# amazon-science/siam-mot

Hardware: AMD Instinct MI355X
Metric: frame-pairs/sec at 720p, 30 active tracks; EMM xcorr HBM GB/s vs peak (higher is better)
Workload: dtype f32 (towers and correlation: fp16x2 operands on MFMA, fp32 accumulate, fp32-equivalent error); 1 GPU; EMM tracker-head frame pair (EMM.forward + EMM.extract_cache) on DLA-34-FPN 720p FPN maps (net input 704x1280, C=128, 5 levels), 30 tracks, one stream per GPU; hot path only: backbone / RPN / box head / solver are outside the timed region; tracks=30, channels=128, rz=15, rx=30, feature_sets=8, feature_bytes_rotated=307281920

## Files before the change

measure/debug/tower_stage_timeline.py:

```python
import json, os, sys
import numpy as np, torch
sys.path.insert(0, os.path.join(os.path.dirname(__file__), "..", "..")); sys.path.insert(0, os.path.join(os.path.dirname(__file__), "..", "..", "tests"))
import golden_inputs as gi
import siammot_amd.ops as ops
dev = "cuda:0"
rs = np.random.RandomState(0)
Pn = gi.predictor_params(rs, 128, np.array([[0, 0, 80, 120]], dtype=np.float32))
P = {k: torch.from_numpy(v).to(dev) for k, v in Pn.items()}
n = int(os.environ.get("TRACKS", "30"))
resp = torch.randn(n, 128, 16, 16, device=dev) * 15
with ops.debug_library(SMOT_TOWER_OCT=2, SMOT_TOWER_BF3=1, SMOT_WINO_ABL=15):
    f = lambda: ops.emm_predictor(resp, P)
    for _ in range(20): f()
    torch.cuda.synchronize()
    grid = (n + 7) // 8 * 8 * 8
    tr = torch.zeros(grid * 64, dtype=torch.int64, device=dev)
    lib = ops.load_library()
    lib.smot_debug_trace(ops._ptr(tr)); f(); torch.cuda.synchronize(); tr.zero_(); f(); torch.cuda.synchronize()
    lib.smot_debug_trace(ops._ptr(None))
t = tr.view(grid, 8, 8).cpu().numpy().astype(np.float64)
t = t[t[:, 0, 5] != 0]
base = t[:, :, 0].min(axis=1)[:, None, None]
rel = (t[:, :, :6] - base)
names = ["before_barrier1", "after_barrier1", "raw_planes_stored", "vector_phase_done", "after_vmcnt0_and_barrier2", "matrix_and_fetches_issued"]
print(json.dumps({"tracks": n, "workgroups": int(t.shape[0]), "slots": names,
                  "mean_cycles_by_wave": {("wave%d" % w): [round(float(x), 0) for x in rel[:, w, :].mean(0)] for w in range(8)}}))
```

measure/debug/tower_wg_spread.py:

```python
import json, os, sys
import numpy as np, torch
sys.path.insert(0, os.path.join(os.path.dirname(__file__), "..", "..")); sys.path.insert(0, os.path.join(os.path.dirname(__file__), "..", "..", "tests"))
import golden_inputs as gi
import siammot_amd.ops as ops
dev = "cuda:0"
rs = np.random.RandomState(0)
P = {k: torch.from_numpy(v).to(dev) for k, v in gi.predictor_params(rs, 128, np.array([[0, 0, 80, 120]], dtype=np.float32)).items()}
for n in [int(t) for t in os.environ.get("TRACKS", "30").split(",")]:
    resp = torch.randn(n, 128, 16, 16, device=dev) * 15
    with ops.debug_library(SMOT_TOWER_OCT=2, SMOT_TOWER_BF3=1):
        f = lambda: ops.emm_predictor(resp, P)
        for _ in range(30): f()
        torch.cuda.synchronize()
        grid = (n + 7) // 8 * 8 * 8
        tr = torch.zeros(grid * 8, dtype=torch.int64, device=dev)
        lib = ops.load_library()
        lib.smot_debug_trace(ops._ptr(tr))
        rows = []
        for rep in range(5):
            tr.zero_(); f(); torch.cuda.synchronize()
            t = tr.view(grid, 8).cpu().numpy().astype(np.float64); t = t[t[:, 5] != 0]
            t0 = t[:, 0].min()
            rows.append({"workgroups": int(t.shape[0]), "start_offset_mean": float((t[:, 0] - t0).mean()), "start_offset_max": float((t[:, 0] - t0).max()),
                         "duration_mean": float((t[:, 5] - t[:, 0]).mean()), "duration_min": float((t[:, 5] - t[:, 0]).min()), "duration_max": float((t[:, 5] - t[:, 0]).max()),
                         "first_start_to_last_end": float(t[:, 5].max() - t0),
                         "phase_max": [float(x) for x in np.diff(t[:, :6], axis=1).max(0)], "phase_p90": [float(x) for x in np.percentile(np.diff(t[:, :6], axis=1), 90, axis=0)]})
        lib.smot_debug_trace(ops._ptr(None))
        ts = []
        for rep in range(3):
            ops.kernel_timer_begin(ops.TIMER_TOWER, 200)
            for _ in range(200): f()
            ms, cnt = ops.kernel_timer_end(ops.TIMER_TOWER)
            ts.append(ms / cnt * 1e3)
    print(json.dumps({"tracks": n, "tower_us": round(min(ts), 2), "launches": rows[-2:]}))
```

measure/lib_ab.py:

```python
import json, os, sys
import torch
sys.path.insert(0, os.path.join(os.path.dirname(os.path.abspath(__file__)), ".."))
import bench
import siammot_amd.ops as ops
from siammot_amd.structures import BoxList
from siammot_amd.emm import EMM
from siammot_amd.config import get_default_cfg
from siammot_amd.track_utils import build_track_utils
dev = torch.device("cuda:0")
base = ops.load_library()
other = ops._open(os.path.abspath(sys.argv[1]), ops._SIGNATURES)
assert other.smot_abi_version() == ops.ABI_VERSION
feats = [bench.synthetic_features(k, dev) for k in range(4)]
n = 30
boxes = bench.synthetic_boxes(n, (1280, 704)).to(dev)
det = BoxList(boxes, (1280, 704), mode="xyxy")
det.add_field("ids", torch.arange(n, device=dev))
det.add_field("labels", torch.ones(n, dtype=torch.int64, device=dev))
cfg = get_default_cfg(channels=bench.CHANNELS)
emm = EMM(cfg, build_track_utils(cfg)).eval()
bench.init_predictor(emm.predictor, boxes.cpu())
emm = emm.to(dev)
ref = None
for rep in range(3):
    for name, lib in (("product", base), ("variant", other)):
        ops._lib = lib
        with torch.no_grad():
            state = emm.extract_cache(feats[3], det)
            def step(k, state):
                z, sr, d = state
                _, res, _ = emm(feats[k % 4], d, sr, template_features=z)
                return emm.extract_cache(feats[k % 4], det), res
            for k in range(100):
                state, res = step(k, state)
            out = torch.cat((res[0].bbox, res[0].get_field("scores")[:, None]), 1).clone()
            ref = out if ref is None else ref
            torch.cuda.synchronize()
            ts = []
            for _ in range(5):
                e0, e1 = torch.cuda.Event(enable_timing=True), torch.cuda.Event(enable_timing=True)
                e0.record()
                for k in range(300):
                    state, res = step(k, state)
                e1.record(); torch.cuda.synchronize()
                ts.append(e0.elapsed_time(e1) / 300 * 1e3)
            r = bench.tracking_loop_throughput(30, dev, feats[:2], steps=400, refine=True)
        print(json.dumps({"library": name, "frame_pair_us": round(min(ts), 2), "bitwise_equal": bool(torch.equal(out, ref)),
                          "loop_refine_ms": round(r["ms_per_frame"], 4)}), flush=True)
ops._lib = base
```

siam-mot_amd/csrc/tower_wino.hip:

```cpp
#include "tower_common.h"
#include "knobs.h"
#include <utility>

namespace smot {

constexpr int W_ROW = 24;
constexpr int W_PLANE = 448;
constexpr int W_STAGE_IC = 8;
constexpr int W_RING = 4;
constexpr int W_BUF = W_STAGE_IC * W_PLANE;
constexpr int W_XOC = 68;
constexpr int W_X_FLOATS = 4 * 2 * 16 * W_XOC;
constexpr int W_PL_OFF = W_X_FLOATS;
constexpr int W_HW_OFF = W_PL_OFF + 16 * T_PLANE;
constexpr int W_ST_OFF = W_HW_OFF + 16 * 36;
constexpr int W_EPI_FLOATS = W_ST_OFF + 32;
constexpr int w_smem_floats(int oct) {
    return (oct * W_EPI_FLOATS > W_RING * W_BUF) ? oct * W_EPI_FLOATS : W_RING * W_BUF;
}
constexpr int W_A_FLOATS = 4 * 4 * 2 * 2 * 256;
constexpr int W_A_SLOT = 4 * 2 * 2 * 256;
constexpr int W_AB_ROW = 4 * 2 * 1024;
static_assert((W_RING * W_BUF + W_A_FLOATS) * 4 <= 160 * 1024, "BF3: ring + A image in one CU's LDS");
static_assert(w_smem_floats(1) * 4 <= 64 * 1024, "OCT = 1: two workgroups per CU, no opt-in needed");
static_assert(w_smem_floats(2) * 4 <= 160 * 1024, "OCT = 2: one workgroup per CU");

__device__ __forceinline__ float tower_pack_scale(unsigned wmax_bits) {
    const int e = (int)((wmax_bits >> 23) & 0xffu);
    if (e == 0 || e == 255) return 1.0f;
    int k = 266 - e;
    k = k < 1 ? 1 : (k > 254 ? 254 : k);
    return __uint_as_float((unsigned)k << 23);
}

__global__ void __launch_bounds__(256)
tower_pack_kernel(const float* __restrict__ wc, const float* __restrict__ wr, int C, float* __restrict__ packed,
                  unsigned* __restrict__ hdr) {
    const int idx = blockIdx.x * 256 + threadIdx.x;
    if (idx >= 2 * C * C) return;
    const int oc = idx / C, ic = idx - oc * C;
    const float* g = (oc < C ? wc + (size_t)oc * C * 9 : wr + (size_t)(oc - C) * C * 9) + (size_t)ic * 9;
    float gg[4][3];
#pragma unroll
    for (int v = 0; v < 3; ++v) {
        const float g0 = g[v], g1 = g[3 + v], g2 = g[6 + v];
        gg[0][v] = g0;
        gg[1][v] = 0.5f * ((g0 + g1) + g2);
        gg[2][v] = 0.5f * ((g0 - g1) + g2);
        gg[3][v] = g2;
    }
    const int tile = oc >> 4, k = ic >> 2, lane = (oc & 15) + 16 * (ic & 3);
    const int nk = C >> 2;
#pragma unroll
    for (int i = 0; i < 4; ++i) {
        float4 u;
        u.x = gg[i][0];
        u.y = 0.5f * ((gg[i][0] + gg[i][1]) + gg[i][2]);
        u.z = 0.5f * ((gg[i][0] - gg[i][1]) + gg[i][2]);
        u.w = gg[i][2];
        *reinterpret_cast<float4*>(packed + ((((size_t)tile * nk + k) * 4 + i) * 64 + lane) * 4) = u;
        if ((C & 31) == 0) {
            unsigned short* hf = reinterpret_cast<unsigned short*>(packed + (size_t)2 * C * C * 16);
            const int kb = ic >> 5, sidx = (ic & 31) >> 2, nkb1 = (C >> 5) + 1;
            const float su = tower_pack_scale(hdr[0]);
            const float uq[4] = {u.x, u.y, u.z, u.w};
#pragma unroll
            for (int q = 0; q < 4; ++q) {
                const int kbp = ((sidx >> 1) <= q) ? kb : kb + 1;
                float r = uq[q] * su;
#pragma unroll
                for (int part = 0; part < 2; ++part) {
                    const _Float16 h = (_Float16)r;
                    r -= (float)h;
                    hf[((((((size_t)tile * nkb1 + kbp) * 4 + i) * 4 + q) * 2 + part) * 64 + lane) * 8 + sidx] =
                        __builtin_bit_cast(unsigned short, h);
                }
            }
            if (idx == 0 && i == 0) reinterpret_cast<float*>(hdr)[1] = 1.0f / su;
        }
    }
}

__global__ void __launch_bounds__(256)
tower_wmax_kernel(const float* __restrict__ wc, const float* __restrict__ wr, int count, unsigned* __restrict__ hdr) {
    float m = 0.0f;
    for (int e = blockIdx.x * 256 + threadIdx.x; e < count; e += gridDim.x * 256) m = fmaxf(m, fmaxf(fabsf(wc[e]), fabsf(wr[e])));
    for (int off = 32; off; off >>= 1) m = fmaxf(m, __shfl_xor(m, off));
    if ((threadIdx.x & 63) == 0) atomicMax(hdr, __float_as_uint(m));
}

__global__ void __launch_bounds__(256)
plane_absmax_kernel(const float* __restrict__ resp, int planes, int hw, float* __restrict__ pm) {
    const int plane = blockIdx.x * 4 + (threadIdx.x >> 6), lane = threadIdx.x & 63;
    if (plane >= planes) return;
    const float* __restrict__ src = resp + (size_t)plane * hw;
    float m = 0.0f;
    for (int e = lane; e < hw; e += 64) m = plane_max_step(m, src[e]);
    m = plane_max_wave(m);
    if (lane == 0) pm[plane] = m;
}

int launch_plane_absmax(const float* resp, int planes, int hw, float* pm, hipStream_t st) {
    hipLaunchKernelGGL(plane_absmax_kernel, dim3((planes + 3) / 4), dim3(256), 0, st, resp, planes, hw, pm);
    return check_launch("predictor towers (plane maxima)");
}

template <int G, int... E>
__device__ __forceinline__ void heads_group(const float (&hw)[9], const float (&a)[36], f32x4& h0, f32x4& h1,
                                            std::integer_sequence<int, E...>) {
    (((E % 2 == 0 ? h0 : h1) = __builtin_amdgcn_mfma_f32_4x4x1f32(hw[(G * 36 + E) / 16], a[E], (E % 2 == 0 ? h0 : h1), 4,
                                                                  (G * 36 + E) % 16, 0)), ...);
}

template <int ABL, int OCT, int BHO = 0, bool BF3 = false>
__global__ void __launch_bounds__(256 * OCT, OCT == 1 ? 2 : 1)
tower_wino_kernel(const float* __restrict__ resp, const float* __restrict__ packed, const float* __restrict__ plane_max,
                  unsigned* __restrict__ zero_words, long long* __restrict__ trace, int N, int C, int cpg, float eps,
                  float* __restrict__ part, TowerParams P) {
    constexpr int NT = 256 * OCT;
    constexpr int NP = 2 / OCT;
    constexpr bool BLOCKED = BHO > 0;
    constexpr int MAP = BLOCKED ? BHO * BHO : 256;
    constexpr int RAW4 = 512 / NT;
    constexpr int RAWB = (W_STAGE_IC * 324 + NT - 1) / NT;
    static_assert(!BLOCKED || (BHO > 16 && BHO <= 32), "four 16 x 16 blocks cover maps of 17 .. 32");
    extern __shared__ __attribute__((aligned(16))) float sm[];
    const int tid = threadIdx.x;
#define W_TRACE(SLOT) \
    if (ABL != 15 && trace && tid == 0) trace[(size_t)blockIdx.x * 8 + (SLOT)] = (long long)__builtin_amdgcn_s_memtime();
    W_TRACE(0)
    if (ABL != 15 && trace && tid == 0) {
        trace[(size_t)blockIdx.x * 8 + 6] = (long long)__builtin_amdgcn_s_getreg(0xF804);
        trace[(size_t)blockIdx.x * 8 + 7] = (long long)__builtin_amdgcn_s_getreg(0xF814);
    }
    const int lane = tid & 63;
    const int wave = __builtin_amdgcn_readfirstlane(tid >> 6);
    const int xi = wave & 3;
    const int nh = wave >> 2;
    const int tiles_per_tower = C >> 4;
    const int tiles = 2 * tiles_per_tower;
    const int wg_per_track = tiles / OCT;
    const int xcd = blockIdx.x & 7, slot = blockIdx.x >> 3;
    const int wg_per_n = BLOCKED ? 4 * wg_per_track : wg_per_track;
    const int n = (slot / wg_per_n) * 8 + xcd;
    const int within = slot % wg_per_n;
    const int blk = BLOCKED ? within / wg_per_track : 0;
    const int oy = BLOCKED ? (blk >> 1) * (BHO - 16) : 0, ox = BLOCKED ? (blk & 1) * (BHO - 16) : 0;
    const int tile0 = (within % wg_per_track) * OCT;
    if (n >= N) return;
    if (zero_words != nullptr && tile0 == 0 && blk == 0 && tid == 0) zero_words[n] = 0u;
    const float* __restrict__ in = resp + (size_t)n * C * MAP;
    const int nk = C >> 2;
    const int nstages = C / W_STAGE_IC;
    const int sub = tid >> 8, ltid = tid & 255;
    const int etile = tile0 + sub;
    const int tower = etile / tiles_per_tower;
    const int oc0 = (etile - tower * tiles_per_tower) * 16;

    auto make_rsrc = [](const float* base) {
        const unsigned long long a = reinterpret_cast<unsigned long long>(base);
        const unsigned lo = __builtin_amdgcn_readfirstlane((unsigned)a);
        const unsigned hi = __builtin_amdgcn_readfirstlane((unsigned)(a >> 32));
        return __builtin_amdgcn_make_buffer_rsrc(reinterpret_cast<void*>(((unsigned long long)hi << 32) | lo), 0,
                                                 0x7fffffff, 0x00020000);
    };
    typedef unsigned u32x4 __attribute__((ext_vector_type(4)));
    auto make_rsrc_sized = [](const float* base, unsigned bytes) {
        const unsigned long long a = reinterpret_cast<unsigned long long>(base);
        const unsigned lo = __builtin_amdgcn_readfirstlane((unsigned)a);
        const unsigned hi = __builtin_amdgcn_readfirstlane((unsigned)(a >> 32));
        return __builtin_amdgcn_make_buffer_rsrc(reinterpret_cast<void*>(((unsigned long long)hi << 32) | lo), 0,
                                                 (int)bytes, 0x00020000);
    };
    const auto rs_in = BLOCKED ? make_rsrc_sized(in, (unsigned)C * MAP * 4u) : make_rsrc(in);
    const auto rs_a = make_rsrc(packed);
    constexpr int NRAW = BLOCKED ? (RAWB + 3) / 4 : RAW4;
    float4 prs[2][NRAW];
    unsigned raw_voff[BLOCKED ? RAWB : RAW4];
    int raw_lds[BLOCKED ? RAWB : RAW4];
    if constexpr (!BLOCKED) {
#pragma unroll
        for (int j = 0; j < RAW4; ++j) {
            const int f = tid + NT * j;
            const int f4 = f & 63;
            raw_voff[j] = (unsigned)((f >> 6) * 256 + f4 * 4) * 4u;
            raw_lds[j] = (f >> 6) * W_PLANE + ((f4 >> 2) + 1) * W_ROW + 1 + (f4 & 3) * 4;
        }
    } else {
#pragma unroll
        for (int j = 0; j < RAWB; ++j) {
            const int e = tid + NT * j;
            const int ch = e / 324, rem = e - ch * 324;
            const int r = rem / 18, c = rem - r * 18;
            const int sy = oy - 1 + r, sx = ox - 1 + c;
            const bool inside = e < W_STAGE_IC * 324 && sy >= 0 && sy < BHO && sx >= 0 && sx < BHO;
            raw_voff[j] = inside ? (unsigned)(ch * MAP + sy * BHO + sx) * 4u : 0x7FFF0000u;
            raw_lds[j] = e < W_STAGE_IC * 324 ? ch * W_PLANE + r * W_ROW + c : (W_STAGE_IC - 1) * W_PLANE + 432 + (tid & 15);
        }
    }
    auto load_raw = [&](int st, float4* pr) {
        const int soff = __builtin_amdgcn_readfirstlane(st * (W_STAGE_IC * MAP * 4));
        if constexpr (!BLOCKED) {
#pragma unroll
            for (int j = 0; j < RAW4; ++j) {
                const u32x4 v = __builtin_bit_cast(u32x4, __builtin_amdgcn_raw_buffer_load_b128(rs_in, raw_voff[j], soff, 0));
                pr[j] = make_float4(__uint_as_float(v.x), __uint_as_float(v.y), __uint_as_float(v.z), __uint_as_float(v.w));
            }
        } else {
            float* f = reinterpret_cast<float*>(pr);
#pragma unroll
            for (int j = 0; j < RAWB; ++j)
                f[j] = __int_as_float(__builtin_amdgcn_raw_buffer_load_b32(rs_in, raw_voff[j], soff, 0));
        }
    };
    typedef int i32x4 __attribute__((ext_vector_type(4)));
    const unsigned long long pin = reinterpret_cast<unsigned long long>(in);
    const i32x4 rs_in_words = {__builtin_amdgcn_readfirstlane((int)(unsigned)pin),
                               __builtin_amdgcn_readfirstlane((int)((unsigned)(pin >> 32) & 0xffffu)),
                               BLOCKED ? (int)((unsigned)C * MAP * 4u) : 0x7fffffff, 0x00020000};
    auto load_raw_asm = [&](int st, float4* pr) __attribute__((always_inline)) {
        const int soff = __builtin_amdgcn_readfirstlane(st * (W_STAGE_IC * MAP * 4));
        if constexpr (!BLOCKED) {
#pragma unroll
            for (int j = 0; j < RAW4; ++j) {
                f32x4 v;
                asm volatile("buffer_load_dwordx4 %0, %1, %2, %3 offen" : "=v"(v) : "v"(raw_voff[j]), "s"(rs_in_words), "s"(soff) : "memory");
                pr[j] = make_float4(v[0], v[1], v[2], v[3]);
            }
        } else {
            float* f = reinterpret_cast<float*>(pr);
#pragma unroll
            for (int j = 0; j < RAWB; ++j)
                asm volatile("buffer_load_dword %0, %1, %2, %3 offen" : "=v"(f[j]) : "v"(raw_voff[j]), "s"(rs_in_words), "s"(soff) : "memory");
        }
    };
    float sv = 1.0f, inv_sv = 1.0f;
    auto store_raw = [&](float* buf, const float4* pr) {
        if constexpr (!BLOCKED) {
#pragma unroll
            for (int j = 0; j < RAW4; ++j) {
                float* d = buf + raw_lds[j];
                d[0] = BF3 ? pr[j].x * sv : pr[j].x;
                d[1] = BF3 ? pr[j].y * sv : pr[j].y;
                d[2] = BF3 ? pr[j].z * sv : pr[j].z;
                d[3] = BF3 ? pr[j].w * sv : pr[j].w;
            }
        } else {
            const float* f = reinterpret_cast<const float*>(pr);
#pragma unroll
            for (int j = 0; j < RAWB; ++j) buf[raw_lds[j]] = BF3 ? f[j] * sv : f[j];
        }
    };
    const unsigned a_voff = (unsigned)lane * 16u;
    const int a_base = __builtin_amdgcn_readfirstlane((int)((((size_t)tile0 * nk) * 4 + xi) * 1024));
    const int a_tile = nk * 4096;
    f32x4 aset[2][2][OCT];
    auto load_a = [&](int st, f32x4 (*dst)[OCT]) {
#pragma unroll
        for (int o = 0; o < OCT; ++o)
#pragma unroll
            for (int k = 0; k < 2; ++k) {
                const int soff = __builtin_amdgcn_readfirstlane(a_base + o * a_tile + (2 * st + k) * 4096);
                dst[k][o] = __builtin_bit_cast(f32x4, __builtin_amdgcn_raw_buffer_load_b128(rs_a, a_voff, soff, 0));
            }
    };

    const int nkb = C >> 5;
    const int ab_block = 4 * W_AB_ROW;
    const int ab_base = __builtin_amdgcn_readfirstlane(2 * C * C * 64 + ((tile0 + nh) * (nkb + 1) * 4 + xi) * W_AB_ROW);
    typedef __attribute__((address_space(3))) float lds_float;
    lds_float* const a_lds = (lds_float*)(sm + W_RING * W_BUF);
    const int al_wave = __builtin_amdgcn_readfirstlane((xi * 2 + nh) * 512);
    const int al_row = __builtin_amdgcn_readfirstlane(xi * 2 * 512);
    const unsigned long long pa = reinterpret_cast<unsigned long long>(packed);
    const i32x4 rs_a_words = {__builtin_amdgcn_readfirstlane((int)(unsigned)pa),
                              __builtin_amdgcn_readfirstlane((int)((unsigned)(pa >> 32) & 0xffffu)), 0x7fffffff, 0x00020000};
    const unsigned a_lds_byte = (unsigned)(size_t)a_lds;
    auto dma_part = [&](int q, int kbp, int part) __attribute__((always_inline)) {
        const int soff = __builtin_amdgcn_readfirstlane(ab_base + (ABL == 12 ? 0 : kbp) * ab_block + (q * 2 + part) * 1024);
        const unsigned dst = __builtin_amdgcn_readfirstlane(a_lds_byte + (unsigned)(q * W_A_SLOT + al_wave + part * 256) * 4u);
        unsigned keep;
        asm volatile("s_mov_b32 %0, m0\n\ts_mov_b32 m0, %1\n\ts_nop 0\n\tbuffer_load_dwordx4 %2, %3, %4 offen lds\n\ts_mov_b32 m0, %0"
                     : "=&s"(keep) : "s"(dst), "v"(a_voff), "s"(rs_a_words), "s"(soff) : "memory");
    };
    auto dma_slot = [&](int q, int kbp) __attribute__((always_inline)) {
        dma_part(q, kbp, 0);
        dma_part(q, kbp, 1);
    };
    auto load_al = [&](int q, u32x4 (*dst)[2]) __attribute__((always_inline)) {
        const float* src = sm + W_RING * W_BUF + q * W_A_SLOT + al_row + lane * 4;
#pragma unroll
        for (int o = 0; o < OCT; ++o)
#pragma unroll
            for (int part = 0; part < 2; ++part)
                dst[o][part] = *reinterpret_cast<const u32x4*>(src + (o * 2 + part) * 256);
    };
    f32x4 acc[OCT][4][2 * NP];
#pragma unroll
    for (int o = 0; o < OCT; ++o)
#pragma unroll
        for (int q = 0; q < 4; ++q)
#pragma unroll
            for (int t = 0; t < 2 * NP; ++t) acc[o][q][t] = (f32x4){0.f, 0.f, 0.f, 0.f};

    load_raw(0, prs[0]);
    load_raw(1, prs[1]);
    if constexpr (BF3) {
        dma_slot(0, 0);
        dma_slot(1, 0);
    }
    if constexpr (!BF3) load_a(0, aset[0]);
    if (ABL == 2 || ABL >= 5) {
#pragma unroll
        for (int o = 0; o < OCT; ++o) {
            aset[1][0][o] = aset[0][0][o];
            aset[1][1][o] = aset[0][1][o];
        }
    }
    float pmv[2] = {0.0f, 0.0f};
    if constexpr (BF3 && ABL != 10) {
        const float* __restrict__ pmsrc = plane_max + (size_t)n * C;
        if (lane < C) pmv[0] = pmsrc[lane];
        if (lane + 64 < C) pmv[1] = pmsrc[lane + 64];
        __builtin_amdgcn_sched_barrier(0);
    }
    {
        float4* z = reinterpret_cast<float4*>(sm);
        for (int e = tid; e < W_RING * W_BUF / 4; e += NT) z[e] = make_float4(0.f, 0.f, 0.f, 0.f);
    }
    float hwv[9];
    auto load_hwv = [&]() __attribute__((always_inline)) {
        const int o = lane & 3, blk = lane >> 2;
        const float* wsrc = (tower == 1) ? P.reg_w + (size_t)o * C * 9
                                         : (o < 2 ? P.cls_w + (size_t)o * C * 9 : P.center_w);
        const bool live = (tower == 1) || (o < 3);
        wsrc += (size_t)oc0 * 9 + blk;
#pragma unroll
        for (int r = 0; r < 9; ++r) hwv[r] = live ? wsrc[r * 16] : 0.0f;
    };
    if constexpr (!BF3) load_hwv();
    if constexpr (BF3 && ABL != 10) {
        float m = fmaxf(pmv[0], pmv[1]);
        for (int c = lane + 128; c < C; c += 64) m = fmaxf(m, plane_max[(size_t)n * C + c]);
        m = plane_max_wave(m);
        const int e = (int)((__float_as_uint(m) >> 23) & 0xffu);
        if (e != 0 && e != 255) {
            int k = 139 - e;
            k = k < -100 ? -100 : (k > 100 ? 100 : k);
            sv = __uint_as_float((unsigned)(127 + k) << 23);
            inv_sv = __uint_as_float((unsigned)(127 - k) << 23);
        }
    }

    __syncthreads();
    if constexpr (BF3) asm volatile("s_waitcnt vmcnt(0)" ::: "memory");
    store_raw(sm, prs[0]);
    store_raw(sm + W_BUF, prs[1]);
    load_raw(min(2, nstages - 1), prs[0]);
    load_raw(min(3, nstages - 1), prs[1]);
    float ga = 0.0f, be = 0.0f;
    if constexpr (!BLOCKED) {
        ga = P.gamma[tower][oc0 + (ltid >> 4)];
        be = P.beta[tower][oc0 + (ltid >> 4)];
    }
    __syncthreads();

    const int row_a = (xi == 0) ? 0 : ((xi == 2) ? 2 : 1);
    const int row_b = (xi == 2) ? 1 : ((xi == 3) ? 3 : 2);
    const int kq = lane >> 4, xl = lane & 15;
    const int patch0 = kq * W_PLANE + (2 * (xl >> 2) + (OCT == 2 ? 8 * nh : 0)) * W_ROW + 4 * (xl & 3);
    int ia = patch0 + row_a * W_ROW, ib = patch0 + row_b * W_ROW;
    asm volatile("" : "+v"(ia), "+v"(ib));

    float rd[NP][6][2];
    float bop[4][2 * NP];
    if (ABL >= 3) {
#pragma unroll
        for (int e = 0; e < 12 * NP; ++e) {
            (&bop[0][0])[e % (8 * NP)] = (float)(lane + e);
            (&rd[0][0][0])[e] = (float)(lane - e);
        }
    }
#define W_READ(BUFI, Q, RD)                                                                      \
    if (ABL != 3 && (ABL < 5 || ABL >= 7)) {                                                     \
        const float* oa = sm + ia + ((BUFI) * W_BUF + (Q) * 4 * W_PLANE);                        \
        const float* ob = sm + ib + ((BUFI) * W_BUF + (Q) * 4 * W_PLANE);                        \
        _Pragma("unroll") for (int p = 0; p < NP; ++p) {             \
            f32x4 a4 = *reinterpret_cast<const f32x4*>(oa + p * 8 * W_ROW);                      \
            f32x2 a2 = *reinterpret_cast<const f32x2*>(oa + p * 8 * W_ROW + 4);                  \
            f32x4 b4 = *reinterpret_cast<const f32x4*>(ob + p * 8 * W_ROW);                      \
            f32x2 b2 = *reinterpret_cast<const f32x2*>(ob + p * 8 * W_ROW + 4);                  \
            if (BF3) asm volatile("" : "+v"(a4), "+v"(a2), "+v"(b4), "+v"(b2));                  \
            RD[p][0][0] = a4[0]; RD[p][0][1] = b4[0];                                            \
            RD[p][1][0] = a4[1]; RD[p][1][1] = b4[1];                                            \
            RD[p][2][0] = a4[2]; RD[p][2][1] = b4[2];                                            \
            RD[p][3][0] = a4[3]; RD[p][3][1] = b4[3];                                            \
            RD[p][4][0] = a2[0]; RD[p][4][1] = b2[0];                                            \
            RD[p][5][0] = a2[1]; RD[p][5][1] = b2[1];                                            \
        }                                                                                        \
    }
#define W_XFORM(RD, BOP)                                                                         \
    if (ABL != 3 && (ABL < 5 || ABL >= 7)) _Pragma("unroll") for (int p = 0; p < NP; ++p) {      \
                     \
        float w[6];                                                                              \
        _Pragma("unroll") for (int c = 0; c < 6; ++c)                                            \
            w[c] = PLUS ? RD[p][c][0] + RD[p][c][1] : RD[p][c][0] - RD[p][c][1];                 \
        BOP[0][2 * p] = w[0] - w[2];                                                             \
        BOP[1][2 * p] = w[1] + w[2];                                                             \
        BOP[2][2 * p] = w[2] - w[1];                                                             \
        BOP[3][2 * p] = w[1] - w[3];                                                             \
        BOP[0][2 * p + 1] = w[2] - w[4];                                                         \
        BOP[1][2 * p + 1] = w[3] + w[4];                                                         \
        BOP[2][2 * p + 1] = w[4] - w[3];                                                         \
        BOP[3][2 * p + 1] = w[3] - w[5];                                                         \
    }
#define W_MFMA(AV, BOP)                                                                          \
    if (ABL != 4) _Pragma("unroll") for (int t = 0; t < 2 * NP; ++t)                             \
        _Pragma("unroll") for (int o = 0; o < OCT; ++o) {                                        \
            acc[o][0][t] = __builtin_amdgcn_mfma_f32_16x16x4f32(AV[o][0], BOP[0][t], acc[o][0][t], 0, 0, 0);   \
            acc[o][1][t] = __builtin_amdgcn_mfma_f32_16x16x4f32(AV[o][1], BOP[1][t], acc[o][1][t], 0, 0, 0);   \
            acc[o][2][t] = __builtin_amdgcn_mfma_f32_16x16x4f32(AV[o][2], BOP[2][t], acc[o][2][t], 0, 0, 0);   \
            acc[o][3][t] = __builtin_amdgcn_mfma_f32_16x16x4f32(AV[o][3], BOP[3][t], acc[o][3][t], 0, 0, 0);   \
        }
#define W_FENCE __builtin_amdgcn_sched_barrier(0);
#define W_STAGE(J)                                                                               \
    {                                                                                            \
        if (ABL != 6) __syncthreads();                                                           \
        if (ABL != 1 && ABL < 5) store_raw(sm + (((J) + 2) & 3) * W_BUF, prs[(J) & 1]);          \
        if (ABL != 1 && ABL < 5) load_raw(min(s0 + (J) + 4, nstages - 1), prs[(J) & 1]);         \
        if (ABL != 2 && ABL < 5) load_a(min(s0 + (J) + 1, nstages - 1), aset[((J) + 1) & 1]);    \
        W_FENCE                                                                                  \
        W_READ((J), 1, rd)                                                      \
        W_MFMA(aset[(J) & 1][0], bop)                                                            \
        W_FENCE                                                                                  \
        W_XFORM(rd, bop)                                                                         \
        W_FENCE                                                                                  \
        W_READ(((J) + 1) & 3, 0, rd)                     \
        W_MFMA(aset[(J) & 1][1], bop)                                                            \
        W_FENCE                                                                                  \
        W_XFORM(rd, bop)                                                                         \
        W_FENCE                                                                                  \
    }
#define W_LOOP                                                                                   \
    W_READ(0, 0, rd)                                                                             \
    W_XFORM(rd, bop)                                                                             \
    W_FENCE                                                                                      \
    for (int s0 = 0; s0 < nstages; s0 += 4) {        \
        W_STAGE(0)                                                                               \
        W_STAGE(1)                                                                               \
        W_STAGE(2)                                                                               \
        W_STAGE(3)                                                                               \
    }
    typedef _Float16 f16x2 __attribute__((ext_vector_type(2)));
    typedef _Float16 f16x4 __attribute__((ext_vector_type(4)));
    typedef _Float16 f16x8 __attribute__((ext_vector_type(8)));
    typedef unsigned u32x2 __attribute__((ext_vector_type(2)));
    u32x4 Bp[2][4][2];
    float rdb[NP][6][2];
    if constexpr (BF3) {
#pragma unroll
        for (int e = 0; e < 16; ++e) (&Bp[0][0][0])[e] = (u32x4){0u, 0u, 0u, 0u};
    }
    const f16x4 negI = __builtin_bit_cast(f16x4, (u32x2){(lane & 3) == 0 ? 0x0000BC00u : ((lane & 3) == 1 ? 0xBC000000u : 0u),
                                                         (lane & 3) == 2 ? 0x0000BC00u : ((lane & 3) == 3 ? 0xBC000000u : 0u)});
#define WB_CVT(D, A, B) D = __builtin_bit_cast(unsigned, __builtin_convertvector((f32x2){A, B}, f16x2));
#define WB_SPLIT(J, BA, BB)                                                                      \
    {                                                                                            \
        f32x4 v4[4];                                                                             \
        unsigned hh[4][2], mm[4][2];                                                             \
        _Pragma("unroll") for (int q = 0; q < 4; ++q) {                                          \
            v4[q] = (f32x4){BA[q][0], BB[q][0], BA[q][1], BB[q][1]};                             \
            WB_CVT(hh[q][0], v4[q][0], v4[q][1]) WB_CVT(hh[q][1], v4[q][2], v4[q][3])            \
        }                                                                                        \
        W_FENCE                                                                                  \
        _Pragma("unroll") for (int q = 0; q < 4; ++q)                                            \
            v4[q] = __builtin_amdgcn_mfma_f32_4x4x4f16(negI, __builtin_bit_cast(f16x4, (u32x2){hh[q][0], hh[q][1]}), v4[q], 0, 0, 0); \
        W_FENCE                                                                                  \
        _Pragma("unroll") for (int q = 0; q < 4; ++q) {                                          \
            WB_CVT(mm[q][0], v4[q][0], v4[q][1]) WB_CVT(mm[q][1], v4[q][2], v4[q][3])            \
        }                                                                                        \
        W_FENCE                                                                                  \
        _Pragma("unroll") for (int q = 0; q < 4; ++q) {                                          \
            Bp[0][q][0][J] = hh[q][0]; Bp[0][q][1][J] = hh[q][1];                                \
            Bp[1][q][0][J] = mm[q][0]; Bp[1][q][1][J] = mm[q][1];                                \
        }                                                                                        \
    }
#define WB_MM(O, Q, T, PA, PB)                                                                   \
    if (ABL != 7) acc[O][Q][T] = __builtin_amdgcn_mfma_f32_16x16x32_f16(__builtin_bit_cast(f16x8, AB[O][PA]), \
                                                          __builtin_bit_cast(f16x8, Bp[PB][Q][T]), acc[O][Q][T], 0, 0, 0);
#define WB_TERM(Q, PA, PB) WB_MM(0, Q, 0, PA, PB) WB_MM(1, Q, 0, PA, PB) WB_MM(0, Q, 1, PA, PB) WB_MM(1, Q, 1, PA, PB)
#define WB_Q(Q)                                                                                  \
    {                                                                                            \
        u32x4 AB[OCT][2];                                                                        \
        load_al(Q, AB);                                                                          \
        WB_QM(Q)                                                                                 \
    }
#define WB_QM(Q)                                                                                 \
    {                                                                                            \
        if (ABL == 7) { _Pragma("unroll") for (int t = 0; t < 2; ++t) _Pragma("unroll") for (int e = 0; e < 4; ++e)  \
            acc[0][Q][t][e] += __uint_as_float(Bp[0][Q][t][e] ^ Bp[1][Q][t][e] ^ AB[0][0][e] ^ AB[1][1][e]); } \
        WB_TERM(Q, 1, 0) WB_TERM(Q, 0, 1) WB_TERM(Q, 0, 0)                                       \
    }
    const float sgn = __uint_as_float(__builtin_amdgcn_readfirstlane(xi == 1 ? 0x3f800000u : 0xbf800000u));
#define WB_XFORM(RD, BOP)                                                                        \
    _Pragma("unroll") for (int p = 0; p < NP; ++p) {                                             \
        float w[6];                                                                              \
        _Pragma("unroll") for (int c = 0; c < 6; ++c) w[c] = __builtin_fmaf(sgn, RD[p][c][1], RD[p][c][0]); \
        BOP[0][2 * p] = w[0] - w[2];                                                             \
        BOP[1][2 * p] = w[1] + w[2];                                                             \
        BOP[2][2 * p] = w[2] - w[1];                                                             \
        BOP[3][2 * p] = w[1] - w[3];                                                             \
        BOP[0][2 * p + 1] = w[2] - w[4];                                                         \
        BOP[1][2 * p + 1] = w[3] + w[4];                                                         \
        BOP[2][2 * p + 1] = w[4] - w[3];                                                         \
        BOP[3][2 * p + 1] = w[3] - w[5];                                                         \
    }
#define WB_STAMP(J, KB, SLOT) if (ABL == 15 && (KB) == 2 && (J) == 1 && trace && lane == 0) \
        trace[((size_t)blockIdx.x * 8 + wave) * 8 + (SLOT)] = (long long)__builtin_amdgcn_s_memtime();
#define WB_STAGE(J, KB)                                                                          \
    {                                                                                            \
         \
        WB_STAMP(J, KB, 0)                                                                       \
        asm volatile("s_barrier" ::: "memory");                                                  \
        WB_STAMP(J, KB, 1)                                                                       \
        store_raw(sm + (((J) + 2) & 3) * W_BUF, prs[(J) & 1]);                                   \
        W_FENCE                                                                                  \
        WB_STAMP(J, KB, 2)                                                                       \
        float ba[4][2 * NP], bb[4][2 * NP];                                                      \
        u32x4 AB[OCT][2];                                                                        \
        WB_XFORM(rd, ba)                                                          \
        W_READ(((J) + 1) & 3, 0, rd)                     \
        WB_XFORM(rdb, bb)                                                       \
        W_READ(((J) + 1) & 3, 1, rdb)                                                            \
        WB_SPLIT(J, ba, bb)                                                                      \
        load_al(J, AB);                                                                          \
        W_FENCE                                                                                  \
        WB_STAMP(J, KB, 3)                                                                       \
                                            \
        asm volatile("s_waitcnt vmcnt(0) lgkmcnt(12)\n\ts_barrier" ::: "memory");                \
        W_FENCE                                                                                  \
        WB_STAMP(J, KB, 4)                                                                       \
         \
        WB_TERM(J, 1, 0)                                                                         \
        W_FENCE                                                                                  \
        if (ABL != 9) load_raw_asm(min(4 * (KB) + (J) + 4, nstages - 1), prs[(J) & 1]);          \
        if (ABL != 9) dma_part(((J) + 2) & 3, (KB) + ((J) >= 2 ? 1 : 0), 0);                     \
        W_FENCE                                                                                  \
        WB_TERM(J, 0, 1)                                                                         \
        W_FENCE                                                                                  \
        if (ABL != 9) dma_part(((J) + 2) & 3, (KB) + ((J) >= 2 ? 1 : 0), 1);                     \
        W_FENCE                                                                                  \
        WB_TERM(J, 0, 0)                                                                         \
        W_FENCE                                                                                  \
        WB_STAMP(J, KB, 5)                                                                       \
    }
#define WB_BLOCK(KB) WB_STAGE(0, KB) WB_STAGE(1, KB) WB_STAGE(2, KB) WB_STAGE(3, KB)
#define WB_LOOP                                                                                  \
    W_READ(0, 0, rd)                                                                             \
    W_READ(0, 1, rdb)                                                                            \
    if (nh == 1) asm volatile("s_barrier" ::: "memory");             \
    if (nkb == 4) {                      \
        WB_BLOCK(0) WB_BLOCK(1) WB_BLOCK(2) WB_BLOCK(3)                                          \
    } else if ((nkb & 1) == 0) {                      \
        for (int kb = 0; kb < nkb; kb += 2) { WB_BLOCK(kb) WB_BLOCK(kb + 1) }                    \
    } else {                                                                                     \
        for (int kb = 0; kb < nkb; ++kb) { WB_BLOCK(kb) }                                        \
    }                                                                                            \
                                                                      \
    asm volatile("s_barrier" ::: "memory");                                                      \
    dma_slot(2, nkb);                                                                            \
    asm volatile("s_barrier" ::: "memory");                                                      \
    WB_Q(0)                                                                                      \
    asm volatile("s_waitcnt vmcnt(0)" ::: "memory");                                             \
     \
    _Pragma("unroll") for (int j = 0; j < NRAW; ++j) asm volatile("" :: "v"(prs[0][j].x), "v"(prs[0][j].y), "v"(prs[0][j].z), "v"(prs[0][j].w), \
                                                                    "v"(prs[1][j].x), "v"(prs[1][j].y), "v"(prs[1][j].z), "v"(prs[1][j].w)); \
    asm volatile("s_barrier\n\ts_barrier" ::: "memory");                                         \
    WB_Q(1)                                                                                      \
    asm volatile("s_barrier\n\ts_barrier" ::: "memory");                                         \
    WB_Q(2)                                                                                      \
    if (nh == 0) asm volatile("s_barrier" ::: "memory");
    W_TRACE(1)
    if constexpr (BF3) {
        static_assert(!BF3 || (OCT == 2 && (ABL == 0 || ABL == 7 || ABL == 9 || ABL == 10 || ABL == 12 || ABL == 15)), "BF3: two-tile workgroups only");
        {
            WB_LOOP
        }
        load_hwv();
    } else if (xi == 1) {
        constexpr bool PLUS = true;
        W_LOOP
    } else {
        constexpr bool PLUS = false;
        W_LOOP
    }
    __syncthreads();
#undef WB_LOOP
#undef WB_STAGE
#undef WB_STAMP
#undef WB_BLOCK
#undef WB_XFORM
#undef WB_Q
#undef WB_QM
#undef WB_TERM
#undef WB_MM
#undef WB_SPLIT
#undef WB_CVT
#undef W_LOOP
#undef W_FENCE
#undef W_STAGE
#undef W_MFMA
#undef W_XFORM
#undef W_READ
    W_TRACE(2)

#pragma unroll
    for (int o = 0; o < OCT; ++o)
#pragma unroll
        for (int t = 0; t < 2 * NP; ++t)
#pragma unroll
            for (int r = 0; r < 4; ++r) {
                const float p0 = (acc[o][0][t][r] + acc[o][1][t][r]) + acc[o][2][t][r];
                const float p1 = (acc[o][1][t][r] - acc[o][2][t][r]) - acc[o][3][t][r];
                float* dst = sm + o * W_EPI_FLOATS + ((xi * 2) * 16 + (kq * 4 + r)) * W_XOC +
                             16 * (t + (OCT == 2 ? 2 * nh : 0)) + xl;
                dst[0] = p0;
                dst[16 * W_XOC] = p1;
            }
    float* X = sm + sub * W_EPI_FLOATS;
    float* planes = X + W_PL_OFF;
    float* chs = X + W_ST_OFF;
    for (int e = ltid; e < 16 * 68; e += 256) {
        const int pl = e / 68, c = e - pl * 68;
        const int row = c < 18 ? 0 : (c < 36 ? 17 : 1 + ((c - 36) >> 1));
        const int col = c < 18 ? c : (c < 36 ? c - 18 : (((c - 36) & 1) ? 17 : 0));
        planes[pl * T_PLANE + row * 18 + col] = 0.0f;
    }
    __syncthreads();

    W_TRACE(3)
    const int ocl = ltid >> 4, x16 = ltid & 15;
    float y[4][2][2];
#pragma unroll
    for (int b = 0; b < 2; ++b) {
        const float* src = X + (b * 16 + ocl) * W_XOC + 4 * x16;
        const f32x4 x0 = *reinterpret_cast<const f32x4*>(src + 0 * 32 * W_XOC);
        const f32x4 x1 = *reinterpret_cast<const f32x4*>(src + 1 * 32 * W_XOC);
        const f32x4 x2 = *reinterpret_cast<const f32x4*>(src + 2 * 32 * W_XOC);
        const f32x4 x3 = *reinterpret_cast<const f32x4*>(src + 3 * 32 * W_XOC);
#pragma unroll
        for (int t = 0; t < 4; ++t) {
            y[t][0][b] = (x0[t] + x1[t]) + x2[t];
            y[t][1][b] = (x1[t] - x2[t]) - x3[t];
        }
    }
    if constexpr (BF3) {
        const float inv_su = packed[(size_t)2 * C * C * 16 + (size_t)tiles * (nkb + 1) * 8192 + 1];
#pragma unroll
        for (int t = 0; t < 4; ++t)
#pragma unroll
            for (int a = 0; a < 2; ++a)
#pragma unroll
                for (int b = 0; b < 2; ++b) y[t][a][b] = (y[t][a][b] * inv_sv) * inv_su;
    }

    if constexpr (BLOCKED) {
        constexpr int OV = 32 - BHO;
        float* __restrict__ cdst = part + ((size_t)n * 2 * C + (size_t)tower * C + oc0 + ocl) * MAP;
#pragma unroll
        for (int t = 0; t < 4; ++t) {
            const int ty = (x16 & 3) + 4 * (x16 >> 3), tx = 2 * t + ((x16 >> 2) & 1);
#pragma unroll
            for (int a = 0; a < 2; ++a)
#pragma unroll
                for (int b = 0; b < 2; ++b) {
                    const int lr = 2 * ty + a, lc = 2 * tx + b;
                    if ((oy == 0 || lr >= OV) && (ox == 0 || lc >= OV)) cdst[(oy + lr) * BHO + ox + lc] = y[t][a][b];
                }
        }
        return;
    }
    const float inv_cnt = 1.0f / (float)(cpg * 256);
    float s = 0.0f;
#pragma unroll
    for (int t = 0; t < 4; ++t) s += (y[t][0][0] + y[t][0][1]) + (y[t][1][0] + y[t][1][1]);
    s = group16_sum(s);
    float mean = 0.0f, var = 0.0f;
    const int g0 = (ocl / cpg) * cpg;
    if (cpg == 4) {
#define W_RL(V, L) __int_as_float(__builtin_amdgcn_readlane(__float_as_int(V), (L)))
        mean = (((0.0f + W_RL(s, 0)) + W_RL(s, 16)) + W_RL(s, 32)) + W_RL(s, 48);
    } else {
        if (x16 == 0) chs[ocl] = s;
        __syncthreads();
        for (int ch = g0; ch < g0 + cpg; ++ch) mean += chs[ch];
    }
    mean *= inv_cnt;
    float sq = 0.0f;
#pragma unroll
    for (int t = 0; t < 4; ++t)
#pragma unroll
        for (int a = 0; a < 2; ++a)
#pragma unroll
            for (int b = 0; b < 2; ++b) {
                const float d = y[t][a][b] - mean;
                sq += d * d;
            }
    sq = group16_sum(sq);
    if (cpg == 4) {
        var = (((0.0f + W_RL(sq, 0)) + W_RL(sq, 16)) + W_RL(sq, 32)) + W_RL(sq, 48);
#undef W_RL
    } else {
        if (x16 == 0) chs[16 + ocl] = sq;
        __syncthreads();
        for (int ch = g0; ch < g0 + cpg; ++ch) var += chs[16 + ch];
    }
    const float rstd = 1.0f / sqrtf(var * inv_cnt + eps);
    {
        float* pl = planes + ocl * T_PLANE;
#pragma unroll
        for (int t = 0; t < 4; ++t) {
            const int ty = (x16 & 3) + 4 * (x16 >> 3), tx = 2 * t + ((x16 >> 2) & 1);
#pragma unroll
            for (int a = 0; a < 2; ++a)
#pragma unroll
                for (int b = 0; b < 2; ++b) {
                    float v = (y[t][a][b] - mean) * rstd * ga + be;
                    pl[(2 * ty + a + 1) * 18 + 2 * tx + b + 1] = relu_nan(v);
                }
        }
    }
    __syncthreads();

    W_TRACE(4)
    {
        const int py = ((ltid >> 6) << 1) + ((ltid >> 5) & 1) + (((ltid >> 4) & 1) << 3), px = ltid & 15;
        const float* pl0 = planes + py * 18 + px;
        f32x4 hacc = {0.0f, 0.0f, 0.0f, 0.0f}, hacc1 = {0.0f, 0.0f, 0.0f, 0.0f};
        float av[2][36];
#define W_HLOAD(G, BUF) _Pragma("unroll") for (int e = 0; e < 36; ++e)                                        \
        av[BUF][e] = pl0[((G) * 4 + e / 9) * T_PLANE + ((e % 9) / 3) * 18 + (e % 9) % 3];
#define W_HMM(G, BUF) heads_group<G>(hwv, av[BUF], hacc, hacc1, std::make_integer_sequence<int, 36>{});
        W_HLOAD(0, 0)
        __builtin_amdgcn_sched_barrier(0);
        W_HLOAD(1, 1)
        __builtin_amdgcn_sched_barrier(0);
        W_HMM(0, 0)
        __builtin_amdgcn_sched_barrier(0);
        W_HLOAD(2, 0)
        __builtin_amdgcn_sched_barrier(0);
        W_HMM(1, 1)
        __builtin_amdgcn_sched_barrier(0);
        W_HLOAD(3, 1)
        __builtin_amdgcn_sched_barrier(0);
        W_HMM(2, 0)
        __builtin_amdgcn_sched_barrier(0);
        W_HMM(3, 1)
#undef W_HMM
#undef W_HLOAD
        hacc[0] += hacc1[0];
        hacc[1] += hacc1[1];
        hacc[2] += hacc1[2];
        hacc[3] += hacc1[3];
        float* __restrict__ dst = part + ((size_t)n * tiles + etile) * 4 * 256 + py * 16 + px;
        dst[0 * 256] = hacc[0];
        dst[1 * 256] = hacc[1];
        dst[2 * 256] = hacc[2];
        dst[3 * 256] = hacc[3];
    }
    W_TRACE(5)
#undef W_TRACE
}

static int tower_tiles_per_workgroup(int N, int C) {
    (void)N;
    (void)C;
    int oct = 2;
    if (knobs().tower_oct == 1 || knobs().tower_oct == 2) oct = knobs().tower_oct;
// ... 146 lines not shown
```

Before: 19420 frame-pairs/s.

## Stream raw tower input planes straight into LDS via buffer_load lds DMA

In the BF3 non-blocked tower path, the raw input planes are no longer staged through VGPRs with load_raw/store_raw. Each wave now issues buffer_load_dwordx4 with the LDS-direct flag into a compact permuted plane layout. Halo columns come from DPP lane shuffles, and the gap rows are zero-filled once. This is meant to remove register pressure, the VGPR-to-LDS store traffic and a barrier per stage, and it folds the sv scale into the transform. The cost is more complex addressing, a permuted epilogue index, a buffer range guard for out-of-bounds reads, and a risk of subtle layout errors.

Result: faster. 19950 frame-pairs/s, median of 6 (+2.7%).

```diff
diff --git a/measure/debug/tower_stage_timeline.py b/measure/debug/tower_stage_timeline.py
--- a/measure/debug/tower_stage_timeline.py
+++ b/measure/debug/tower_stage_timeline.py
@@ -22,6 +22,6 @@
 t = t[t[:, 0, 5] != 0]
 base = t[:, :, 0].min(axis=1)[:, None, None]
 rel = (t[:, :, :6] - base)
-names = ["before_barrier1", "after_barrier1", "raw_planes_stored", "vector_phase_done", "after_vmcnt0_and_barrier2", "matrix_and_fetches_issued"]
+names = ["before_barrier1", "after_barrier1", "behind_barrier1_no_store", "vector_phase_done", "after_vmcnt0_and_barrier2", "matrix_and_fetches_issued"]
 print(json.dumps({"tracks": n, "workgroups": int(t.shape[0]), "slots": names,
                   "mean_cycles_by_wave": {("wave%d" % w): [round(float(x), 0) for x in rel[:, w, :].mean(0)] for w in range(8)}}))
diff --git a/measure/debug/tower_wg_spread.py b/measure/debug/tower_wg_spread.py
--- a/measure/debug/tower_wg_spread.py
+++ b/measure/debug/tower_wg_spread.py
@@ -24,6 +24,7 @@
             rows.append({"workgroups": int(t.shape[0]), "start_offset_mean": float((t[:, 0] - t0).mean()), "start_offset_max": float((t[:, 0] - t0).max()),
                          "duration_mean": float((t[:, 5] - t[:, 0]).mean()), "duration_min": float((t[:, 5] - t[:, 0]).min()), "duration_max": float((t[:, 5] - t[:, 0]).max()),
                          "first_start_to_last_end": float(t[:, 5].max() - t0),
+                         "phase_mean": [round(float(x)) for x in np.diff(t[:, :6], axis=1).mean(0)],
                          "phase_max": [float(x) for x in np.diff(t[:, :6], axis=1).max(0)], "phase_p90": [float(x) for x in np.percentile(np.diff(t[:, :6], axis=1), 90, axis=0)]})
         lib.smot_debug_trace(ops._ptr(None))
         ts = []
diff --git a/measure/lib_ab.py b/measure/lib_ab.py
--- a/measure/lib_ab.py
+++ b/measure/lib_ab.py
@@ -22,7 +22,7 @@
 bench.init_predictor(emm.predictor, boxes.cpu())
 emm = emm.to(dev)
 ref = None
-for rep in range(3):
+for rep in range(int(sys.argv[2]) if len(sys.argv) > 2 else 3):
     for name, lib in (("product", base), ("variant", other)):
         ops._lib = lib
         with torch.no_grad():
diff --git a/siam-mot_amd/csrc/tower_wino.hip b/siam-mot_amd/csrc/tower_wino.hip
--- a/siam-mot_amd/csrc/tower_wino.hip
+++ b/siam-mot_amd/csrc/tower_wino.hip
@@ -9,6 +9,10 @@
 constexpr int W_STAGE_IC = 8;
 constexpr int W_RING = 4;
 constexpr int W_BUF = W_STAGE_IC * W_PLANE;
+constexpr int D_PLANE = 320;
+constexpr int D_GAP_LO = 256 + 48;
+constexpr int D_GAP_HI = 256;
+constexpr int D_BUF = W_STAGE_IC * D_PLANE;
 constexpr int W_XOC = 68;
 constexpr int W_X_FLOATS = 4 * 2 * 16 * W_XOC;
 constexpr int W_PL_OFF = W_X_FLOATS;
@@ -120,6 +124,7 @@
     constexpr int NT = 256 * OCT;
     constexpr int NP = 2 / OCT;
     constexpr bool BLOCKED = BHO > 0;
+    constexpr bool DMA = BF3 && !BLOCKED;
     constexpr int MAP = BLOCKED ? BHO * BHO : 256;
     constexpr int RAW4 = 512 / NT;
     constexpr int RAWB = (W_STAGE_IC * 324 + NT - 1) / NT;
@@ -215,9 +220,13 @@
     };
     typedef int i32x4 __attribute__((ext_vector_type(4)));
     const unsigned long long pin = reinterpret_cast<unsigned long long>(in);
+    const unsigned long long in_left = (unsigned long long)(N - n) * (unsigned)C * (MAP * 4ull);
     const i32x4 rs_in_words = {__builtin_amdgcn_readfirstlane((int)(unsigned)pin),
                                __builtin_amdgcn_readfirstlane((int)((unsigned)(pin >> 32) & 0xffffu)),
-                               BLOCKED ? (int)((unsigned)C * MAP * 4u) : 0x7fffffff, 0x00020000};
+                               BLOCKED ? (int)((unsigned)C * MAP * 4u)
+                                       : (DMA ? __builtin_amdgcn_readfirstlane((int)(in_left < 0x7fffffffull ? in_left : 0x7fffffffull))
+                                              : 0x7fffffff),
+                               0x00020000};
     auto load_raw_asm = [&](int st, float4* pr) __attribute__((always_inline)) {
         const int soff = __builtin_amdgcn_readfirstlane(st * (W_STAGE_IC * MAP * 4));
         if constexpr (!BLOCKED) {
@@ -287,6 +296,16 @@
         dma_part(q, kbp, 0);
         dma_part(q, kbp, 1);
     };
+    const unsigned pl_voff = (unsigned)((((((lane >> 2) & 3) << 1) | ((lane >> 4) & 1) | ((lane >> 5) << 3)) * 4 + (lane & 3)) * 16);
+    const int pl_soff = __builtin_amdgcn_readfirstlane(wave * 1024);
+    const unsigned pl_dst = __builtin_amdgcn_readfirstlane((unsigned)(size_t)(lds_float*)sm + (unsigned)(wave * D_PLANE) * 4u);
+    auto dma_plane = [&](int st, int slot) __attribute__((always_inline)) {
+        const int soff = __builtin_amdgcn_readfirstlane(st * (W_STAGE_IC * 256 * 4) + pl_soff);
+        const unsigned dst = __builtin_amdgcn_readfirstlane(pl_dst + (unsigned)(slot * D_BUF) * 4u);
+        unsigned keep;
+        asm volatile("s_mov_b32 %0, m0\n\ts_mov_b32 m0, %1\n\ts_nop 0\n\tbuffer_load_dwordx4 %2, %3, %4 offen lds\n\ts_mov_b32 m0, %0"
+                     : "=&s"(keep) : "s"(dst), "v"(pl_voff), "s"(rs_in_words), "s"(soff) : "memory");
+    };
     auto load_al = [&](int q, u32x4 (*dst)[2]) __attribute__((always_inline)) {
         const float* src = sm + W_RING * W_BUF + q * W_A_SLOT + al_row + lane * 4;
 #pragma unroll
@@ -303,8 +322,14 @@
 #pragma unroll
             for (int t = 0; t < 2 * NP; ++t) acc[o][q][t] = (f32x4){0.f, 0.f, 0.f, 0.f};
 
-    load_raw(0, prs[0]);
-    load_raw(1, prs[1]);
+    if constexpr (DMA) {
+        dma_plane(0, 0);
+        dma_plane(1, 1);
+        dma_plane(2, 2);
+    } else {
+        load_raw(0, prs[0]);
+        load_raw(1, prs[1]);
+    }
     if constexpr (BF3) {
         dma_slot(0, 0);
         dma_slot(1, 0);
@@ -324,7 +349,10 @@
         if (lane + 64 < C) pmv[1] = pmsrc[lane + 64];
         __builtin_amdgcn_sched_barrier(0);
     }
-    {
+    if constexpr (DMA) {
+        static_assert(W_RING * W_STAGE_IC * 16 == NT, "one 16-byte piece of the gaps per thread");
+        *reinterpret_cast<float4*>(sm + (tid >> 4) * D_PLANE + 256 + (tid & 15) * 4) = make_float4(0.f, 0.f, 0.f, 0.f);
+    } else {
         float4* z = reinterpret_cast<float4*>(sm);
         for (int e = tid; e < W_RING * W_BUF / 4; e += NT) z[e] = make_float4(0.f, 0.f, 0.f, 0.f);
     }
@@ -352,12 +380,17 @@
         }
     }
 
-    __syncthreads();
-    if constexpr (BF3) asm volatile("s_waitcnt vmcnt(0)" ::: "memory");
-    store_raw(sm, prs[0]);
-    store_raw(sm + W_BUF, prs[1]);
-    load_raw(min(2, nstages - 1), prs[0]);
-    load_raw(min(3, nstages - 1), prs[1]);
+    const float sv_s = __uint_as_float(__builtin_amdgcn_readfirstlane(__float_as_uint(sv)));
+    if constexpr (!DMA) {
+        __syncthreads();
+        if constexpr (BF3) asm volatile("s_waitcnt vmcnt(0)" ::: "memory");
+        store_raw(sm, prs[0]);
+        store_raw(sm + W_BUF, prs[1]);
+        load_raw(min(2, nstages - 1), prs[0]);
+        load_raw(min(3, nstages - 1), prs[1]);
+    } else {
+        asm volatile("s_waitcnt vmcnt(0)" ::: "memory");
+    }
     float ga = 0.0f, be = 0.0f;
     if constexpr (!BLOCKED) {
         ga = P.gamma[tower][oc0 + (ltid >> 4)];
@@ -370,6 +403,14 @@
     const int kq = lane >> 4, xl = lane & 15;
     const int patch0 = kq * W_PLANE + (2 * (xl >> 2) + (OCT == 2 ? 8 * nh : 0)) * W_ROW + 4 * (xl & 3);
     int ia = patch0 + row_a * W_ROW, ib = patch0 + row_b * W_ROW;
+    if constexpr (DMA) {
+        auto d_row = [](int r) {
+            return r < 0 ? D_GAP_LO : (r > 15 ? D_GAP_HI : 16 * ((((r >> 3) & 1) << 3) | ((r & 1) << 2) | ((r >> 1) & 3)));
+        };
+        const int r0 = 2 * ((xl & 3) + 4 * nh) - 1;
+        ia = kq * D_PLANE + d_row(r0 + row_a) + 4 * (xl >> 2);
+        ib = kq * D_PLANE + d_row(r0 + row_b) + 4 * (xl >> 2);
+    }
     asm volatile("" : "+v"(ia), "+v"(ib));
 
     float rd[NP][6][2];
@@ -502,11 +543,32 @@
         WB_TERM(Q, 1, 0) WB_TERM(Q, 0, 1) WB_TERM(Q, 0, 0)                                       \
     }
     const float sgn = __uint_as_float(__builtin_amdgcn_readfirstlane(xi == 1 ? 0x3f800000u : 0xbf800000u));
+#define WB_DPP(V, CTRL) __int_as_float(__builtin_amdgcn_update_dpp(0, __float_as_int(V), (CTRL), 0xf, 0xf, true))
+#define D_READ(BUFI, Q, RD)                                                                      \
+    {                                                                                            \
+        const float* oa = sm + ia + ((BUFI) * D_BUF + (Q) * 4 * D_PLANE);                        \
+        const float* ob = sm + ib + ((BUFI) * D_BUF + (Q) * 4 * D_PLANE);                        \
+        f32x4 a4 = *reinterpret_cast<const f32x4*>(oa);      \
+        f32x4 b4 = *reinterpret_cast<const f32x4*>(ob);            \
+        asm volatile("" : "+v"(a4), "+v"(b4));                                                   \
+        _Pragma("unroll") for (int c = 0; c < 4; ++c) { RD[0][c + 1][0] = a4[c]; RD[0][c + 1][1] = b4[c]; } \
+    }
+#define WB_READ(BUFI, Q, RD) if constexpr (DMA) D_READ(BUFI, Q, RD) else { W_READ(BUFI, Q, RD) }
 #define WB_XFORM(RD, BOP)                                                                        \
     _Pragma("unroll") for (int p = 0; p < NP; ++p) {                                             \
         float w[6];                                                                              \
-        _Pragma("unroll") for (int c = 0; c < 6; ++c) w[c] = __builtin_fmaf(sgn, RD[p][c][1], RD[p][c][0]); \
-        BOP[0][2 * p] = w[0] - w[2];                                                             \
+        if constexpr (DMA) {                                                                     \
+            const f32x2 w12 = __builtin_elementwise_fma((f32x2){sgn, sgn}, (f32x2){RD[p][1][1], RD[p][2][1]},     \
+                                                        (f32x2){RD[p][1][0], RD[p][2][0]}) * (f32x2){sv_s, sv_s}; \
+            const f32x2 w34 = __builtin_elementwise_fma((f32x2){sgn, sgn}, (f32x2){RD[p][3][1], RD[p][4][1]},     \
+                                                        (f32x2){RD[p][3][0], RD[p][4][0]}) * (f32x2){sv_s, sv_s}; \
+            w[1] = w12[0]; w[2] = w12[1]; w[3] = w34[0]; w[4] = w34[1];                          \
+            w[0] = WB_DPP(w[4], 0x114);                     \
+            w[5] = WB_DPP(w[1], 0x104);                     \
+        } else {                                                                                 \
+            _Pragma("unroll") for (int c = 0; c < 6; ++c) w[c] = __builtin_fmaf(sgn, RD[p][c][1], RD[p][c][0]); \
+        }                                                                                        \
+        BOP[0][2 * p] = w[0] - w[2];                                                         \
         BOP[1][2 * p] = w[1] + w[2];                                                             \
         BOP[2][2 * p] = w[2] - w[1];                                                             \
         BOP[3][2 * p] = w[1] - w[3];                                                             \
@@ -523,27 +585,30 @@
         WB_STAMP(J, KB, 0)                                                                       \
         asm volatile("s_barrier" ::: "memory");                                                  \
         WB_STAMP(J, KB, 1)                                                                       \
-        store_raw(sm + (((J) + 2) & 3) * W_BUF, prs[(J) & 1]);                                   \
-        W_FENCE                                                                                  \
-        WB_STAMP(J, KB, 2)                                                                       \
+        if constexpr (!DMA) store_raw(sm + (((J) + 2) & 3) * W_BUF, prs[(J) & 1]);               \
+        W_FENCE                                                                                  \
+        WB_STAMP(J, KB, 2)                                    \
         float ba[4][2 * NP], bb[4][2 * NP];                                                      \
         u32x4 AB[OCT][2];                                                                        \
         WB_XFORM(rd, ba)                                                          \
-        W_READ(((J) + 1) & 3, 0, rd)                     \
+        WB_READ(((J) + 1) & 3, 0, rd)                    \
         WB_XFORM(rdb, bb)                                                       \
-        W_READ(((J) + 1) & 3, 1, rdb)                                                            \
+        WB_READ(((J) + 1) & 3, 1, rdb)                                                           \
         WB_SPLIT(J, ba, bb)                                                                      \
         load_al(J, AB);                                                                          \
         W_FENCE                                                                                  \
         WB_STAMP(J, KB, 3)                                                                       \
-                                            \
-        asm volatile("s_waitcnt vmcnt(0) lgkmcnt(12)\n\ts_barrier" ::: "memory");                \
+                                \
+        if constexpr (DMA) asm volatile("s_waitcnt vmcnt(0)\n\ts_barrier" ::: "memory");         \
+        else asm volatile("s_waitcnt vmcnt(0) lgkmcnt(12)\n\ts_barrier" ::: "memory");           \
         W_FENCE                                                                                  \
         WB_STAMP(J, KB, 4)                                                                       \
          \
         WB_TERM(J, 1, 0)                                                                         \
         W_FENCE                                                                                  \
-        if (ABL != 9) load_raw_asm(min(4 * (KB) + (J) + 4, nstages - 1), prs[(J) & 1]);          \
+        if constexpr (DMA) {                            \
+            if (ABL != 9 && 4 * (KB) + (J) + 3 < 4 * nkb) dma_plane(4 * (KB) + (J) + 3, ((J) + 3) & 3); \
+        } else if (ABL != 9) load_raw_asm(min(4 * (KB) + (J) + 4, nstages - 1), prs[(J) & 1]);   \
         if (ABL != 9) dma_part(((J) + 2) & 3, (KB) + ((J) >= 2 ? 1 : 0), 0);                     \
         W_FENCE                                                                                  \
         WB_TERM(J, 0, 1)                                                                         \
@@ -556,8 +621,8 @@
     }
 #define WB_BLOCK(KB) WB_STAGE(0, KB) WB_STAGE(1, KB) WB_STAGE(2, KB) WB_STAGE(3, KB)
 #define WB_LOOP                                                                                  \
-    W_READ(0, 0, rd)                                                                             \
-    W_READ(0, 1, rdb)                                                                            \
+    WB_READ(0, 0, rd)                                                                            \
+    WB_READ(0, 1, rdb)                                                                           \
     if (nh == 1) asm volatile("s_barrier" ::: "memory");             \
     if (nkb == 4) {                      \
         WB_BLOCK(0) WB_BLOCK(1) WB_BLOCK(2) WB_BLOCK(3)                                          \
@@ -573,8 +638,10 @@
     WB_Q(0)                                                                                      \
     asm volatile("s_waitcnt vmcnt(0)" ::: "memory");                                             \
      \
-    _Pragma("unroll") for (int j = 0; j < NRAW; ++j) asm volatile("" :: "v"(prs[0][j].x), "v"(prs[0][j].y), "v"(prs[0][j].z), "v"(prs[0][j].w), \
-                                                                    "v"(prs[1][j].x), "v"(prs[1][j].y), "v"(prs[1][j].z), "v"(prs[1][j].w)); \
+    if constexpr (!DMA) {                                                                        \
+        _Pragma("unroll") for (int j = 0; j < NRAW; ++j) asm volatile("" :: "v"(prs[0][j].x), "v"(prs[0][j].y), "v"(prs[0][j].z), "v"(prs[0][j].w), \
+                                                                        "v"(prs[1][j].x), "v"(prs[1][j].y), "v"(prs[1][j].z), "v"(prs[1][j].w)); \
+    }                                                                                            \
     asm volatile("s_barrier\n\ts_barrier" ::: "memory");                                         \
     WB_Q(1)                                                                                      \
     asm volatile("s_barrier\n\ts_barrier" ::: "memory");                                         \
@@ -600,6 +667,9 @@
 #undef WB_STAMP
 #undef WB_BLOCK
 #undef WB_XFORM
+#undef WB_READ
+#undef D_READ
+#undef WB_DPP
 #undef WB_Q
 #undef WB_QM
 #undef WB_TERM
@@ -623,7 +693,7 @@
                 const float p0 = (acc[o][0][t][r] + acc[o][1][t][r]) + acc[o][2][t][r];
                 const float p1 = (acc[o][1][t][r] - acc[o][2][t][r]) - acc[o][3][t][r];
                 float* dst = sm + o * W_EPI_FLOATS + ((xi * 2) * 16 + (kq * 4 + r)) * W_XOC +
-                             16 * (t + (OCT == 2 ? 2 * nh : 0)) + xl;
+                             16 * (t + (OCT == 2 ? 2 * nh : 0)) + (DMA ? ((xl & 3) << 2) | (xl >> 2) : xl);
                 dst[0] = p0;
                 dst[16 * W_XOC] = p1;
             }
```
